# uc-vision/smart-tree

Measured on AMD Instinct MI355X. Metric: points/sec end-to-end (voxelize->sparse-UNet->skeleton), 1M-pt tree, higher is better.
Workload: dtype f32

## Files before the change

include/smarttree_hip.h:

```cpp
#ifndef SMARTTREE_HIP_H
#define SMARTTREE_HIP_H

#include <stdint.h>

#ifdef __cplusplus
extern "C" {
#endif

int st_version(void);
#define ST_SKELETON_STATS_ENTRIES 16
#define ST_SKELETON_TUNING_ENTRIES 24
int st_abi_entries(int what);
const char* st_last_error(void);
int64_t st_query_workspace(int op, int64_t a, int64_t b, int64_t c);

int64_t st_scan_workspace_bytes(int64_t n);
int st_scan_u32(const uint32_t* in, uint32_t* out, int64_t n, uint32_t* total, void* ws, int64_t ws_bytes, void* stream);
int64_t st_sort_workspace_bytes(int64_t n);
int st_sort_pairs_u32(uint32_t* keys, uint32_t* vals, int64_t n, int key_bits, void* ws, int64_t ws_bytes, void* stream);

int64_t st_voxelize_workspace_bytes(int64_t n_points, int max_blocks, int64_t max_voxels);
int st_voxelize_blocks(const float* xyz, const float* rgb, int64_t n, double voxel_size, double block_size,
                       double buffer_size, int min_points, int max_blocks, int64_t max_voxels, float* feats,
                       int32_t* coords, uint8_t* mask, int64_t* point_index, float* block_centres,
// ... 17 lines not shown
                              int32_t* up_order ,
                              void* stream);

int st_sparse_conv_fwd(const float* x0, int c0, const float* x1, int cin, const int32_t* nbr, int K, int64_t n_out,
                       const float* w, int cout, const float* scale, const float* shift, const float* residual,
                       int relu, float* y, const int32_t* row_order ,
                       void* stream, int64_t nbr_stride );
int st_sparse_conv_mfma_fwd(const float* x0, int c0, const float* x1, int cin, const int32_t* nbr, int K, int64_t n_out,
                            const float* wp, int cout, const float* scale, const float* shift, const float* residual,
                            int relu, float* y, const int32_t* row_order ,
                            void* stream, int64_t nbr_stride ,
                            int variant );
int st_sparse_conv_b3_fwd(const float* x0, int c0, const float* x1, int cin, const int32_t* nbr, int K, int64_t n_out, const void* wq,
                          int cout, const float* scale, const float* shift, const float* residual, int relu, float* y,
                          const int32_t* row_order, void* stream, int64_t nbr_stride, int variant);
int st_sparse_conv_f16_fwd(const void* x0, int c0, const void* x1, int cin, const int32_t* nbr, int K, int64_t n_out,
                           const void* w, int cout, const float* scale, const float* shift, const void* residual, int relu,
                           void* y, int in_half, int out_half, const int32_t* row_order, void* stream, int64_t nbr_stride );

int64_t st_brick_pyramid_workspace_bytes(int64_t n0, int n_blocks, int coord_bound, int depth, const int64_t* caps);
int st_brick_pyramid(const int32_t* coords0 , int64_t n0, int n_blocks ,
                     int coord_bound , int depth, const int32_t* blk_seg ,
                     int nseg, const int64_t* caps ,
                     int32_t* order0 , int32_t* const* coords_out ,
                     int32_t* const* subm , int32_t* const* down ,
                     int32_t* const* up , int32_t* const* up_order ,
                     int64_t* counts_host , void* ws, int64_t ws_bytes, void* stream);
int st_head_param_floats(void);
int st_pointwise_mlp_heads(const float* x, int64_t n, const float* params, float* radius, float* direction,
                           float* class_l, float* medial_vector , int64_t* class_idx , void* stream);
// ... 157 lines not shown
```

smart_tree_amd/_lib.py:

```python
from __future__ import annotations

import ctypes
from ctypes import c_double, c_float, c_int, c_int64, c_void_p
from pathlib import Path

import torch

_PKG = Path(__file__).resolve().parent
LIB_PATH = _PKG / "libsmarttree_hip.so"

_LIB = None
_ALLOW_HOST_POINTERS = False

P = c_void_p
I64 = c_int64

SIGNATURES = {
    "st_version": (c_int, []),
    "st_abi_entries": (c_int, [c_int]),
    "st_last_error": (ctypes.c_char_p, []),
    "st_scan_workspace_bytes": (I64, [I64]),
    "st_scan_u32": (c_int, [P, P, I64, P, P, I64, P]),
    "st_sort_workspace_bytes": (I64, [I64]),
    "st_sort_pairs_u32": (c_int, [P, P, I64, c_int, P, I64, P]),
# ... 1 lines not shown
    "st_voxelize_blocks": (c_int, [P, P, I64, c_double, c_double, c_double, c_int, c_int, I64, P, P, P, P, P,
                                   ctypes.POINTER(I64), ctypes.POINTER(I64), P, I64, P]),
    "st_hash_capacity": (I64, [I64]),
    "st_build_coord_hash": (c_int, [P, I64, P, P, I64, P]),
    "st_build_subm_rulebook": (c_int, [P, I64, P, P, I64, P, P]),
    "st_strided_workspace_bytes": (I64, [I64]),
    "st_spatial_order_workspace_bytes": (I64, [I64]),
    "st_spatial_order": (c_int, [P, I64, P, P, I64, P]),
    "st_move_rows": (c_int, [P, c_int, P, I64, P, c_int, P]),
    "st_build_strided_outputs": (c_int, [P, I64, I64, P, P, P, I64, ctypes.POINTER(I64), ctypes.POINTER(ctypes.c_int32),
                                         P, I64, P]),
    "st_build_strided_rulebook": (c_int, [P, I64, P, P, I64, P, I64, P, P, I64, ctypes.POINTER(ctypes.c_int32), P, P, P, P]),
    "st_sparse_conv_fwd": (c_int, [P, c_int, P, c_int, P, c_int, I64, P, c_int, P, P, P, c_int, P, P, P, I64]),
    "st_sparse_conv_mfma_fwd": (c_int, [P, c_int, P, c_int, P, c_int, I64, P, c_int, P, P, P, c_int, P, P, P, I64, c_int]),
    "st_sparse_conv_b3_fwd": (c_int, [P, c_int, P, c_int, P, c_int, I64, P, c_int, P, P, P, c_int, P, P, P, I64, c_int]),
    "st_sparse_conv_f16_fwd": (c_int, [P, c_int, P, c_int, P, c_int, I64, P, c_int, P, P, P, c_int, P, c_int, c_int, P, P, I64]),
    "st_brick_pyramid_workspace_bytes": (I64, [I64, c_int, c_int, c_int, ctypes.POINTER(I64)]),
    "st_brick_pyramid": (c_int, [P, I64, c_int, c_int, c_int, P, c_int, ctypes.POINTER(I64), P, ctypes.POINTER(P), ctypes.POINTER(P),
                                 ctypes.POINTER(P), ctypes.POINTER(P), ctypes.POINTER(P), ctypes.POINTER(I64), P, I64, P]),
    "st_head_param_floats": (c_int, []),
    "st_pointwise_mlp_heads": (c_int, [P, I64, P, P, P, P, P, P, P]),
    "st_knn_workspace_bytes": (I64, [I64]),
    "st_knn_radius": (c_int, [P, I64, P, I64, c_int, c_float, P, c_int, c_float, P, P, P, I64, P]),
    "st_medial_points": (c_int, [P, P, I64, P, P, P]),
    "st_centre_cloud": (c_int, [P, I64, P, P, I64, P]),
    "st_make_edges_workspace_bytes": (I64, [I64]),
    "st_make_edges": (c_int, [P, P, I64, c_int, P, P, ctypes.POINTER(I64), P, I64, P]),
    "st_connected_components_workspace_bytes": (c_int64, [c_int64]),
    "st_connected_components": (c_int, [P, I64, I64, P, P, I64, P]),
    "st_component_layout_workspace_bytes": (I64, [I64]),
# ... 48 lines not shown
    "st_bn_stats": (c_int, [P, c_int, I64, c_int, P, P, I64, P]),
    "st_bn_apply": (c_int, [P, c_int, I64, c_int, P, P, P, P, P, P]),
    "st_bn_backward_stats": (c_int, [P, P, c_int, I64, c_int, P, P, P, P, I64, P]),
    "st_bn_backward_apply": (c_int, [P, P, c_int, I64, c_int, P, P, P, P, P, P, P]),
    "st_skeleton_components": (c_int, [c_int, P, P, I64, P, P, P, P, P, P, c_float, c_int, c_int, P, P, P, P, P, P, P, P,
                                       P, P, ctypes.POINTER(I64), P, I64, P]),
}


ENQUEUE_ONLY = frozenset({
    "st_version", "st_abi_entries", "st_last_error", "st_scan_workspace_bytes", "st_sort_workspace_bytes", "st_voxelize_workspace_bytes",
    "st_hash_capacity", "st_strided_workspace_bytes", "st_head_param_floats", "st_knn_workspace_bytes",
    "st_make_edges_workspace_bytes", "st_connected_components_workspace_bytes", "st_component_layout_workspace_bytes",
    "st_component_csr_workspace_bytes", "st_assemble_workspace_bytes", "st_skeleton_workspace_bytes",
    "st_build_coord_hash", "st_build_subm_rulebook", "st_build_strided_rulebook", "st_sparse_conv_fwd",
    "st_sparse_conv_mfma_fwd", "st_sparse_conv_b3_fwd", "st_sparse_conv_f16_fwd", "st_pointwise_mlp_heads", "st_medial_points", "st_centre_cloud",
    "st_connected_components", "st_component_csr", "st_post_process", "st_knn_radius", "st_brick_pyramid_workspace_bytes",
    "st_centre_cloud_seg", "st_centre_cloud_box_seg", "st_voxelize_workspace_bytes_seg", "st_build_strided_rulebook_seg", "st_knn_workspace_bytes_seg",
    "st_knn_radius_seg", "st_skeleton_workspace_bytes_seg", "st_post_process_seg", "st_radius_count_seg",
    "st_voxelize_cloud_workspace_bytes", "st_loss_workspace_bytes", "st_spatial_order_workspace_bytes", "st_spatial_order", "st_connected_components_knn", "st_component_csr_knn", "st_component_csr_knn_workspace_bytes", "st_move_rows",
    "st_loss_backward", "st_sparse_conv_wgrad_workspace_bytes", "st_sparse_conv_wgrad",
    "st_sparse_conv_h_fwd", "st_sparse_conv_wgrad_h_workspace_bytes", "st_sparse_conv_wgrad_h", "st_move_rows_h",
    "st_bn_workspace_bytes", "st_bn_stats", "st_bn_apply", "st_bn_backward_stats", "st_bn_backward_apply",
    "st_sample_tubes_workspace_bytes", "st_sample_tubes_fill", "st_skeleton_match_workspace_bytes", "st_skeleton_match",
})


NOWAIT_VARIANTS = ("st_make_edges", "st_assemble_branches", "st_make_edges_seg")


class _Bound:
# ... 79 lines not shown
```

smart_tree_amd/csrc/sparse_conv.hip:

```cpp
#include "st_common.h"

#define CONV_BLOCK 256

typedef _Float16 st_h;
typedef _Float16 st_v4h __attribute__((ext_vector_type(4)));
__device__ __forceinline__ float4 conv_load4(const float* p) { return *reinterpret_cast<const float4*>(p); }
__device__ __forceinline__ float4 conv_load4(const st_h* p) {
    const st_v4h v = *reinterpret_cast<const st_v4h*>(p);
    return make_float4((float)v.x, (float)v.y, (float)v.z, (float)v.w);
}
__device__ __forceinline__ void conv_store4(float* p, float a, float b, float c, float d) { *reinterpret_cast<float4*>(p) = make_float4(a, b, c, d); }
__device__ __forceinline__ void conv_store4(st_h* p, float a, float b, float c, float d) {
    *reinterpret_cast<st_v4h*>(p) = st_v4h{(st_h)a, (st_h)b, (st_h)c, (st_h)d};
}

__device__ __forceinline__ uint32_t conv_live_offsets(int32_t entry, int K) {
    const uint32_t tag = (uint32_t)entry >> 28;
    if (!(tag & 8u) || K != 27) return 0xffffffffu;
    const uint32_t ax[3] = {(tag & 4u) ? 5u : 2u, (tag & 2u) ? 5u : 2u, (tag & 1u) ? 5u : 2u};
    uint32_t live = 0;
#pragma unroll
    for (int k = 0; k < 27; k++)
        if (((ax[0] >> (k / 9)) & (ax[1] >> ((k / 3) % 3)) & (ax[2] >> (k % 3))) & 1u) live |= 1u << k;
    return live;
}
#define CONV_ROW_MASK 0x0fffffff

template <int CIN, int COT, class TIN = float, class TOUT = float>
__global__ void __launch_bounds__(CONV_BLOCK) k_sparse_conv(const TIN* __restrict__ x0, int c0,
                                                            const TIN* __restrict__ x1, const int32_t* __restrict__ nbr,
                                                            int K, int64_t n_out, int64_t nstride, const float* __restrict__ w, int cout,
                                                            const float* __restrict__ scale, const float* __restrict__ shift,
                                                            const float* __restrict__ residual, int relu,
                                                            TOUT* __restrict__ y, const int32_t* __restrict__ row_order) {
    const int co_tiles = cout / COT;
    const int co0 = (int)(blockIdx.x % co_tiles) * COT;
    const int64_t pos = (int64_t)(blockIdx.x / co_tiles) * CONV_BLOCK + threadIdx.x;
    const bool active = pos < n_out;
    const int32_t entry = active && row_order ? row_order[pos] : 0;
    const int64_t o = active && row_order ? (int64_t)(entry & CONV_ROW_MASK) : pos;
    const uint32_t live = conv_live_offsets(entry, K);
    const int c1 = CIN - c0;
    float acc[COT];
#pragma unroll
    for (int c = 0; c < COT; c++) acc[c] = 0.0f;

    if (CIN % 4 == 0 && CIN <= 16) {
        constexpr int G = CIN <= 8 ? 9 : 3, Q = CIN / 4;
        for (int k0 = 0; k0 < K; k0 += G) {
            int idx[G];
            float4 v[G][Q];
#pragma unroll
            for (int j = 0; j < G; j++) {
                const int k = k0 + j;
                idx[j] = -1;
                if (k < K && active && ((live >> k) & 1u)) idx[j] = nbr ? nbr[(int64_t)k * nstride + o] : (int)o;
            }
#pragma unroll
            for (int j = 0; j < G; j++)
                if (idx[j] >= 0) {
#pragma unroll
                    for (int q = 0; q < Q; q++) {
                        const int ci = 4 * q;
                        const TIN* row = ci < c0 ? x0 + (int64_t)idx[j] * c0 + ci : x1 + (int64_t)idx[j] * c1 + (ci - c0);
                        v[j][q] = conv_load4(row);
                    }
                }
#pragma unroll
            for (int j = 0; j < G; j++) {
                if (idx[j] < 0) continue;
                const float* __restrict__ wk = w + (int64_t)(k0 + j) * CIN * cout + co0;
#pragma unroll
                for (int q = 0; q < Q; q++) {
                    const float xs[4] = {v[j][q].x, v[j][q].y, v[j][q].z, v[j][q].w};
#pragma unroll
                    for (int jj = 0; jj < 4; jj++)
#pragma unroll
                        for (int c = 0; c < COT; c++) acc[c] = fmaf(xs[jj], wk[(4 * q + jj) * cout + c], acc[c]);
                }
            }
        }
    } else
    for (int k = 0; k < K; k++) {
        int idx = -1;
        if (active && ((live >> k) & 1u)) idx = nbr ? nbr[(int64_t)k * nstride + o] : (int)o;
        if (idx < 0) continue;
        const float* __restrict__ wk = w + (int64_t)k * CIN * cout + co0;
        if (CIN % 4 == 0) {
#pragma unroll 2
            for (int ci = 0; ci < CIN; ci += 4) {
                const TIN* row = ci < c0 ? x0 + (int64_t)idx * c0 + ci : x1 + (int64_t)idx * c1 + (ci - c0);
                const float4 v = conv_load4(row);
                const float xs[4] = {v.x, v.y, v.z, v.w};
#pragma unroll
                for (int j = 0; j < 4; j++)
#pragma unroll
                    for (int c = 0; c < COT; c++) acc[c] = fmaf(xs[j], wk[(ci + j) * cout + c], acc[c]);
            }
        } else {
            for (int ci = 0; ci < CIN; ci++) {
// ... 8 lines not shown
    for (int c = 0; c < COT; c++) {
        float v = acc[c];
        if (scale) v = fmaf(v, scale[co0 + c], shift[co0 + c]);
        if (residual) v += residual[o * cout + co0 + c];
        if (relu) v = v > 0.0f ? v : 0.0f;
        acc[c] = v;
    }
    TOUT* out = y + o * cout + co0;
    if (COT % 4 == 0) {
#pragma unroll
        for (int c = 0; c < COT; c += 4) conv_store4(out + c, acc[c], acc[c + 1], acc[c + 2], acc[c + 3]);
    } else {
#pragma unroll
        for (int c = 0; c < COT; c++) out[c] = (TOUT)acc[c];
    }
}

__global__ void __launch_bounds__(CONV_BLOCK) k_sparse_conv_any(const float* __restrict__ x0, int c0, const float* __restrict__ x1, int cin,
                                                                const int32_t* __restrict__ nbr, int K, int64_t n_out, int64_t nstride,
                                                                const float* __restrict__ w, int cout, const float* __restrict__ scale,
                                                                const float* __restrict__ shift, const float* __restrict__ residual, int relu,
                                                                float* __restrict__ y, const int32_t* __restrict__ row_order) {
    const int64_t pos = (int64_t)blockIdx.x * CONV_BLOCK + threadIdx.x;
    if (pos >= n_out) return;
    const int co0 = (int)blockIdx.y * 4, nco = cout - co0 < 4 ? cout - co0 : 4;
    const int32_t entry = row_order ? row_order[pos] : 0;
    const int64_t o = row_order ? (int64_t)(entry & CONV_ROW_MASK) : pos;
    const uint32_t live = conv_live_offsets(entry, K);
    const int c1 = cin - c0;
    float acc[4] = {0.0f, 0.0f, 0.0f, 0.0f};
// ... 18 lines not shown

struct ConvArgs {
    const void* x0;
    int c0;
    const void* x1;
    const int32_t* nbr;
    int K;
    int64_t n_out, nstride;
    const void* w;
    const float *scale, *shift;
    const void* residual;
    int relu;
    void* y;
    const int32_t* row_order;
    hipStream_t stream;
};

static int conv_check_args(ConvArgs* a, int cin) {
    if (a->nstride <= 0) a->nstride = a->n_out;
    ST_REQUIRE(a->K >= 1 && (a->nbr != nullptr || a->K == 1), "conv: a NULL neighbour table means pointwise (K = 1)");
    ST_REQUIRE(a->c0 > 0 && a->c0 <= cin && (a->c0 == cin || a->x1 != nullptr), "conv: bad concat split");
    ST_REQUIRE((a->scale == nullptr) == (a->shift == nullptr), "conv: scale and shift go together");
    return ST_OK;
}

template <int CIN, int COT, class TIN = float, class TOUT = float>
static int conv_launch(const ConvArgs& a, int cout) {
    int64_t blocks = st_div_up(a.n_out, CONV_BLOCK) * (cout / COT);
    hipLaunchKernelGGL((k_sparse_conv<CIN, COT, TIN, TOUT>), dim3((unsigned)blocks), dim3(CONV_BLOCK), 0, a.stream, (const TIN*)a.x0, a.c0,
                       (const TIN*)a.x1, a.nbr, a.K, a.n_out, a.nstride, (const float*)a.w, cout, a.scale, a.shift, (const float*)a.residual,
// ... 73 lines not shown
    static constexpr int CHUNK = 32, PLANES = 1;
    typedef st_v8h Row;
    static __device__ __forceinline__ Row no_row() { return Row{}; }
    static __device__ __forceinline__ Row load_row(const T* row) { return *reinterpret_cast<const st_v8h*>(row); }
    static __device__ __forceinline__ A fragment(const Row& r) { return r; }
    static __device__ __forceinline__ B load_b(const W* wc, int) { return *wc; }
    static __device__ __forceinline__ void mma(const A& a, const B& b, st_v4f& d) { d = __builtin_amdgcn_mfma_f32_16x16x32_f16(a, b, d, 0, 0, 0); }
};

#define MF_PARAMS(T, W)                                                                                                               \
    const T *__restrict__ x0, int c0, const T *__restrict__ x1, const int32_t *__restrict__ nbr, int K, int64_t n_out, int64_t nstride, \
        const W *__restrict__ w, const float *__restrict__ scale, const float *__restrict__ shift, const T *__restrict__ residual,     \
        int relu, T *__restrict__ y, const int32_t *__restrict__ row_order
#define MF_ARGS x0, c0, x1, nbr, K, n_out, nstride, w, scale, shift, residual, relu, y, row_order

template <class OP, int CIN, int COUT, int RT, bool LDSW>
__device__ __forceinline__ void conv_rule_gemm(MF_PARAMS(typename OP::T, typename OP::W)) {
    typedef typename OP::T T;
    typedef typename OP::W W;
    constexpr bool PAIR = CIN == 16 && OP::CHUNK == 32;
    constexpr int CT = COUT / 16, NC = PAIR ? 1 : CIN / OP::CHUNK, LCH = OP::CHUNK / 4;
    constexpr int PLANE = 4 * COUT, WSTEP = NC * OP::PLANES * PLANE;
    __shared__ W wl[LDSW ? WSTEP : 1];
    const int tid = threadIdx.x, lane = tid & 63, wave = tid >> 6;
    const int i16 = lane & 15, g = lane >> 4;
    const int64_t obase = ((int64_t)blockIdx.x * (MF_BLOCK / 64) + wave) * (16 * RT);
    const int c1 = CIN - c0;
    st_v4f acc[RT][CT];
#pragma unroll
    for (int t = 0; t < RT; t++)
#pragma unroll
        for (int ct = 0; ct < CT; ct++) acc[t][ct] = st_v4f{0.0f, 0.0f, 0.0f, 0.0f};
// ... 50 lines not shown
        const float sc = scale ? scale[ch] : 1.0f, sh = scale ? shift[ch] : 0.0f;
#pragma unroll
        for (int t = 0; t < RT; t++)
#pragma unroll
            for (int r = 0; r < 4; r++) {
                const int64_t pos = obase + t * 16 + g * 4 + r;
                if (pos >= n_out) continue;
                const int64_t o = row_order ? (int64_t)(row_order[pos] & CONV_ROW_MASK) : pos;
                float v = acc[t][ct][r];
                if (scale) v = fmaf(v, sc, sh);
                if (residual) v += (float)residual[o * COUT + ch];
                if (relu) v = v > 0.0f ? v : 0.0f;
                y[o * COUT + ch] = (T)v;
            }
    }
}

template <int CIN, int COUT, int RT, bool LDSW>
__global__ void __launch_bounds__(MF_BLOCK) k_sparse_conv_mfma(MF_PARAMS(float, float4)) { conv_rule_gemm<MfF32, CIN, COUT, RT, LDSW>(MF_ARGS); }
template <int CIN, int COUT, int RT>
__global__ void __launch_bounds__(MF_BLOCK) k_sparse_conv_mfma_b3(MF_PARAMS(float, uint4)) { conv_rule_gemm<MfB3, CIN, COUT, RT, false>(MF_ARGS); }
template <int COUT, int RT>
__global__ void __launch_bounds__(MF_BLOCK) k_sparse_conv_mfma_b3_c16(MF_PARAMS(float, uint4)) { conv_rule_gemm<MfB3, 16, COUT, RT, false>(MF_ARGS); }
template <int CIN, int COUT, int RT>
__global__ void __launch_bounds__(MF_BLOCK) k_sparse_conv_mfma_f16x(MF_PARAMS(st_h, st_v8h)) { conv_rule_gemm<MfF16, CIN, COUT, RT, false>(MF_ARGS); }
template <int COUT, int RT>
__global__ void __launch_bounds__(MF_BLOCK) k_sparse_conv_mfma_f16x_c16(MF_PARAMS(st_h, st_v8h)) { conv_rule_gemm<MfF16, 16, COUT, RT, false>(MF_ARGS); }

template <class T, class W>
using mf_kernel_t = void (*)(MF_PARAMS(T, W));
template <int CIN, int COUT, int RT>
static mf_kernel_t<float, uint4> b3_kernel() {
    if constexpr (CIN == 16) return k_sparse_conv_mfma_b3_c16<COUT, RT>;
    else return k_sparse_conv_mfma_b3<CIN, COUT, RT>;
}
template <int CIN, int COUT, int RT>
static mf_kernel_t<st_h, st_v8h> f16x_kernel() {
    if constexpr (CIN == 16) return k_sparse_conv_mfma_f16x_c16<COUT, RT>;
    else return k_sparse_conv_mfma_f16x<CIN, COUT, RT>;
}

template <class T, class W>
static int mf_launch(mf_kernel_t<T, W> kernel, int rt, const ConvArgs& a) {
    hipLaunchKernelGGL(kernel, dim3((unsigned)st_div_up(a.n_out, (MF_BLOCK / 64) * 16 * rt)), dim3(MF_BLOCK), 0, a.stream, (const T*)a.x0, a.c0,
                       (const T*)a.x1, a.nbr, a.K, a.n_out, a.nstride, (const W*)a.w, a.scale, a.shift, (const T*)a.residual, a.relu, (T*)a.y,
                       a.row_order);
    ST_CHECK_LAUNCH();
    return ST_OK;
}

static int conv_row_tiles(const ConvArgs& a) { return a.n_out >= (a.row_order == nullptr ? 56000 : 300000) ? 2 : 1; }

template <int CIN, int COUT>
static int conv_launch_mfma(const ConvArgs& a, int v) {
    if (v == 0) v = (a.row_order == nullptr && a.n_out >= 150000) ? 18 : 1;
    switch (v) {
        case 1: return mf_launch(k_sparse_conv_mfma<CIN, COUT, 1, false>, 1, a);
        case 2: return mf_launch(k_sparse_conv_mfma<CIN, COUT, 2, false>, 2, a);
        case 4: return mf_launch(k_sparse_conv_mfma<CIN, COUT, 4, false>, 4, a);
        case 17: return mf_launch(k_sparse_conv_mfma<CIN, COUT, 1, true>, 1, a);
        default: return mf_launch(k_sparse_conv_mfma<CIN, COUT, 2, true>, 2, a);
// ... 8 lines not shown
    ST_REQUIRE((cin % 32 == 0 || (cin == 16 && c0 == cin)) && cout % 16 == 0 && c0 % 8 == 0,
               "conv(b3): Cin % 32 (or Cin = 16 without concat), Cout % 16 and a concat split % 8 are required");
    if (n_out <= 0) return ST_OK;
    const int rt = variant == 1 || variant == 2 ? variant : conv_row_tiles(a);
#define B3_CASE(CI, CO) \
    if (cin == CI && cout == CO) return rt == 2 ? mf_launch(b3_kernel<CI, CO, 2>(), 2, a) : mf_launch(b3_kernel<CI, CO, 1>(), 1, a);
    B3_CASE(16, 16)
    B3_CASE(16, 32)
    B3_CASE(32, 16)
    B3_CASE(32, 32)
    B3_CASE(32, 64)
    B3_CASE(64, 32)
    B3_CASE(64, 64)
#undef B3_CASE
    st_set_error("conv(b3): no kernel instance for cin=%d cout=%d", cin, cout);
    return ST_ERR_INVALID;
}

extern "C" int st_sparse_conv_f16_fwd(const void* x0, int c0, const void* x1, int cin, const int32_t* nbr, int K, int64_t n_out,
                                      const void* w, int cout, const float* scale, const float* shift, const void* residual,
                                      int relu, void* y, int in_half, int out_half, const int32_t* row_order, void* stream_,
                                      int64_t nbr_stride) {
    ConvArgs a = {x0, c0, x1, nbr, K, n_out, nbr_stride, w, scale, shift, residual, relu, y, row_order, (hipStream_t)stream_};
    ST_TRY(conv_check_args(&a, cin));
    ST_REQUIRE(in_half || out_half, "conv(f16): neither side is half precision -- use st_sparse_conv_fwd");
    if (n_out <= 0) return ST_OK;
    if (in_half && out_half) {
        ST_REQUIRE(cin % 16 == 0 && cout % 16 == 0 && c0 % 16 == 0, "conv(f16): channels and concat split must be multiples of 16");
        const int rt = conv_row_tiles(a);
#define F16X_CASE(CI, CO) \
// ... 60 lines not shown
    CONV_CASE(16, 8, 8)
    CONV_CASE(16, 16, 16)
    CONV_CASE(16, 32, 16)
    CONV_CASE(32, 16, 16)
    CONV_CASE(32, 32, 16)
    CONV_CASE(32, 64, 16)
    CONV_CASE(64, 32, 16)
    CONV_CASE(64, 64, 16)
#undef CONV_CASE
    hipLaunchKernelGGL(k_sparse_conv_any, dim3((unsigned)st_div_up(n_out, CONV_BLOCK), (unsigned)st_div_up(cout, 4)), dim3(CONV_BLOCK), 0, a.stream, x0, c0,
                       x1, cin, nbr, K, n_out, a.nstride, w, cout, scale, shift, residual, relu, y, row_order);
    ST_CHECK_LAUNCH();
    return ST_OK;
}

#define HEAD_W1 0
#define HEAD_S1 64
#define HEAD_T1 72
#define HEAD_W2 80
#define HEAD_S2 112
#define HEAD_T2 116
#define HEAD_W3 120
#define HEAD_STRIDE 132

template <int NOUT>
__device__ __forceinline__ void head_eval(const float* __restrict__ p, const float* x, float* out) {
    float h1[8], h2[4];
#pragma unroll
    for (int co = 0; co < 8; co++) {
        float a = 0.0f;
// ... 60 lines not shown
```

smart_tree_amd/model/model.py:

```python
from __future__ import annotations

import contextlib

from typing import Dict, Mapping

import numpy as np
import torch

from . import sparse_ops as ops
from .. import profiling

BN_EPS = 1e-4


def _conv_weight(t: torch.Tensor) -> torch.Tensor:
    cout, cin = t.shape[0], t.shape[-1]
    return t.reshape(cout, -1, cin).permute(1, 2, 0).contiguous().float()


class _Affine:

    def __init__(self, sd: Mapping[str, torch.Tensor], prefix: str, device):
        g = sd[prefix + ".weight"].double()
        b = sd[prefix + ".bias"].double()
# ... 37 lines not shown
                        self.wp16[name] = ops.mfma_weight16_half(self.w[name])
            elif key.endswith(".running_mean") and "_head." not in key:
                p = key[: -len(".running_mean")]
                self.bn[p] = _Affine(sd, p, self.device)
        self.generic_heads = not self._heads_are_standard(sd)
        self.head_params = None if self.generic_heads else self._pack_heads(sd).to(self.device)
        if self.generic_heads:
            self.head_layers = {}
            for name in ("radius_head", "direction_head", "class_head"):
                mat = lambda i: sd[f"{name}.sequence.{i}.weight"].reshape(sd[f"{name}.sequence.{i}.weight"].shape[0], -1).T.contiguous().float()
                self.head_layers[name] = [(mat(0).unsqueeze(0).to(self.device), _Affine(sd, f"{name}.sequence.1", self.device)),
                                          (mat(3).unsqueeze(0).to(self.device), _Affine(sd, f"{name}.sequence.4", self.device)),
                                          (mat(6).unsqueeze(0).to(self.device), None)]
        self.use_bricks = True
        self.spatial_order = True
        self.trace = None

    def eval(self):
        return self

    def to(self, device):
        return self if torch.device(device) == self.device else Smart_Tree(self._state, device, self.fp16)

    @staticmethod
    def _heads_are_standard(sd) -> bool:
        for name, nout in (("radius_head", 1), ("direction_head", 3), ("class_head", 2)):
            shapes = [tuple(sd[f"{name}.sequence.{i}.weight"].reshape(sd[f"{name}.sequence.{i}.weight"].shape[0], -1).shape) for i in (0, 3, 6)]
            if shapes != [(8, 8), (4, 8), (nout, 4)]:
                return False
        return True
# ... 29 lines not shown
            s2, t2 = affine(4)
            w3 = torch.zeros(12, dtype=torch.float64)
            w3[: 4 * nout] = mat(6).reshape(-1)
            blocks.append(torch.cat([mat(0).reshape(-1), s1, t1, mat(3).reshape(-1), s2, t2, w3]))
        return torch.cat(blocks).float().contiguous()

    def _conv(self, name, x, nbr, n_out, x1=None, bn=None, residual=None, relu=False, row_order=None):
        a = self.bn[bn] if bn else None
        out_half = self.fp16 and self.w[name].shape[2] % 16 == 0
        return ops.sparse_conv(x, self.w[name], nbr, n_out, x1=x1, scale=a.scale if a else None,
                               shift=a.shift if a else None, residual=residual, relu=relu,
                               wp=self.wp.get(name) if self.use_mfma else None, out_half=out_half,
                               wp16=self.wp16.get(name), row_order=row_order,
                               wq=self.wq.get(name) if self.use_mfma and self.use_b3 and not self.fp16 else None)

    def _res_block(self, prefix, x, nbr, x1=None):
        n = x.shape[0]
        h = self._conv(prefix + ".sequence.0", x, nbr, n, x1=x1, bn=prefix + ".sequence.1", relu=True)
        ident = self._conv(prefix + ".identity.0", x, None, n, x1=x1) if x1 is not None else x
        return self._conv(prefix + ".sequence.3", h, nbr, n, bn=prefix + ".sequence.4", residual=ident, relu=True)

    def _ublock(self, prefix, x, pyr, level):
        x = self._res_block(prefix + ".Head", x, pyr.subm[level])
        self._record(f"head{level}", x)
        if level == self.depth:
            return x
        n_fine, n_coarse = x.shape[0], pyr.coords[level + 1].shape[0]
        z = self._conv(prefix + ".Encode.sequence.0", x, pyr.down[level], n_coarse, bn=prefix + ".Encode.sequence.1",
                       relu=True)
        self._record(f"enc{level}", z)
        z = self._ublock(prefix + ".U", z, pyr, level + 1)
        d = self._conv(prefix + ".Decode.sequence.0", z, pyr.up[level], n_fine, bn=prefix + ".Decode.sequence.1",
                       relu=True, row_order=pyr.up_order[level] if pyr.up_order else None)
        self._record(f"dec{level}", d)
        x = self._res_block(prefix + ".Tail", x, pyr.subm[level], x1=d)
        self._record(f"tail{level}", x)
        return x

    def _record(self, name, x):
        if self.trace is not None:
            self.trace[name] = x

    def features(self, sparse_input):
        coords = sparse_input.indices.contiguous()
        feats = sparse_input.features.contiguous().float()
        blk_seg, n_seg = getattr(sparse_input, "blk_seg", None), getattr(sparse_input, "n_seg", 1)
        reorder = self.spatial_order and self.trace is None and coords.shape[0] > 1
        hint = getattr(sparse_input, "brick_hint", None)
        bricks = ops.brick_pyramid(coords, self.depth, hint[0], hint[1], blk_seg, n_seg) if reorder and hint and self.use_bricks else None
        if bricks is not None:
            pyr, order = bricks
            feats = ops.move_rows(feats, order)
        else:
            order = ops.spatial_order(coords) if reorder else None
            if order is not None:
                coords, feats = ops.move_rows(coords, order), ops.move_rows(feats, order)
            pyr = ops.build_pyramid(coords, self.depth, blk_seg, n_seg)
        gate = getattr(self, "conv_gate", None)
        with (gate() if gate is not None else contextlib.nullcontext()), profiling.kernel_family("k_sparse_conv* (one forward pass)"):
            x = self._conv("input_conv.sequence.0", feats, None, feats.shape[0], bn="input_conv.sequence.1", relu=True)
            self._record("input", x)
            x = self._ublock("UNet", x, pyr, 0)
        if order is not None:
            x = ops.move_rows(x, order, scatter=True)
        return x

    def forward(self, sparse_input) -> Dict[str, torch.Tensor]:
        x = self.features(sparse_input)
        radius, direction, class_l, _, _ = self._generic_heads(x, False) if self.generic_heads else ops.mlp_heads(x, self.head_params)
        return {"radius": radius, "direction": direction, "class_l": class_l}

    __call__ = forward

    def forward_fused_tail(self, sparse_input):
        x = self.features(sparse_input)
        return self._generic_heads(x, True) if self.generic_heads else ops.mlp_heads(x, self.head_params, with_tail=True)
```

smart_tree_amd/model/sparse_ops.py:

```python
from __future__ import annotations

import ctypes
from dataclasses import dataclass, field
from typing import List, Optional

import torch

from .. import _lib, profiling


@dataclass
class CoordHash:
    keys: torch.Tensor
    vals: torch.Tensor
    cap: int


def build_coord_hash(coords: torch.Tensor) -> CoordHash:
    L = _lib.lib()
    n = coords.shape[0]
    cap = L.st_hash_capacity(n)
    keys = torch.empty(cap, dtype=torch.int64, device=coords.device)
    vals = torch.empty(cap, dtype=torch.int32, device=coords.device)
    _lib.check(L.st_build_coord_hash(_lib.ptr(coords), n, _lib.ptr(keys), _lib.ptr(vals), cap, _lib.stream(coords.device)))
# ... 282 lines not shown
    elif wp is not None and mfma_eligible(cin, cout, c0) and not big_16:
        entry, wt, name, tail = L.st_sparse_conv_mfma_fwd, wp, f"k_sparse_conv_mfma<{cin},{cout}>", (int(MFMA_VARIANT),)
    else:
        entry, wt, name = L.st_sparse_conv_fwd, w, f"k_sparse_conv<{cin},{cout}>"
    esz_in, esz_out = (2 if in_half else 4), (2 if out_half else 4)
    y = torch.empty((n_out, cout), dtype=torch.float16 if out_half else torch.float32, device=x0.device)
    nbytes = (lambda: (_pair_count(nbr) if nbr is not None else n_out) * (cin * esz_in + (4 if nbr is not None else 0))
              + n_out * cout * esz_out) if profiling.enabled() else 0
    nflops = (lambda: 2.0 * (_pair_count(nbr) if nbr is not None else n_out) * cin * cout) if profiling.enabled() else 0
    with profiling.kernel(name + ("" if nbr is not None else " k1"), nbytes, nflops):
        _lib.check(entry(_lib.ptr(x0), c0, _lib.ptr(x1), cin, nbr_ptr, K, n_out, _lib.ptr(wt), cout, _lib.ptr(scale), _lib.ptr(shift),
                         _lib.ptr(residual), int(relu), _lib.ptr(y), *mid, _lib.ptr(row_order), _lib.stream(x0.device), nbr_stride, *tail))
    return y


_pairs_cache = {}


def _pair_count(nbr: torch.Tensor) -> int:
    key = (id(nbr), profiling.generation())
    if key not in _pairs_cache:
        if len(_pairs_cache) > 4096:
            _pairs_cache.clear()
        _pairs_cache[key] = int((nbr >= 0).sum().item())
    return _pairs_cache[key]


def mlp_heads(x: torch.Tensor, params: torch.Tensor, with_tail: bool = False):
    L = _lib.lib()
    n, dev = x.shape[0], x.device
# ... 11 lines not shown
```

Measured before the change: 937.4 million.

## Fuse Tail identity projection into first conv and fold input gather into input conv

Adds fused kernels in which the Tail residual block's 1x1 identity projection of the concatenated (skip, decoded) features is computed inside the first submanifold conv kernel, for both the vector and b3 MFMA paths. It also adds an input-conv kernel that reads the unpermuted features through the spatial order instead of running a separate move_rows. Together these remove extra launches and re-reads of the concatenated rows. The cost is more register pressure and longer kernels, and the fused path is only taken on the b3/MFMA fp32 path when no trace is recorded.

Result: no change. 938.9 million, median of 4 (+0.2%).

```diff
diff --git a/include/smarttree_hip.h b/include/smarttree_hip.h
--- a/include/smarttree_hip.h
+++ b/include/smarttree_hip.h
@@ -55,6 +55,15 @@
 int st_sparse_conv_b3_fwd(const float* x0, int c0, const float* x1, int cin, const int32_t* nbr, int K, int64_t n_out, const void* wq,
                           int cout, const float* scale, const float* shift, const float* residual, int relu, float* y,
                           const int32_t* row_order, void* stream, int64_t nbr_stride, int variant);
+int st_sparse_conv_tail_fwd(const float* x0, int c0, const float* x1, int cin, const int32_t* nbr, int K, int64_t n_out,
+                            const float* w, int cout, const float* scale, const float* shift, const float* residual, int relu,
+                            float* y, const int32_t* row_order, void* stream, int64_t nbr_stride, const float* w_ident, float* y_ident);
+int st_sparse_conv_tail_b3_fwd(const float* x0, int c0, const float* x1, int cin, const int32_t* nbr, int K, int64_t n_out,
+                               const void* wq, int cout, const float* scale, const float* shift, const float* residual, int relu,
+                               float* y, const int32_t* row_order, void* stream, int64_t nbr_stride, int variant,
+                               const void* wq_ident, float* y_ident);
+int st_sparse_conv_input_fwd(const float* x0, int cin, int64_t n_out, const float* w, int cout, const float* scale,
+                             const float* shift, int relu, float* y, const int32_t* in_order, void* stream);
 int st_sparse_conv_f16_fwd(const void* x0, int c0, const void* x1, int cin, const int32_t* nbr, int K, int64_t n_out,
                            const void* w, int cout, const float* scale, const float* shift, const void* residual, int relu,
                            void* y, int in_half, int out_half, const int32_t* row_order, void* stream, int64_t nbr_stride );
diff --git a/smart_tree_amd/_lib.py b/smart_tree_amd/_lib.py
--- a/smart_tree_amd/_lib.py
+++ b/smart_tree_amd/_lib.py
@@ -39,6 +39,9 @@
     "st_sparse_conv_fwd": (c_int, [P, c_int, P, c_int, P, c_int, I64, P, c_int, P, P, P, c_int, P, P, P, I64]),
     "st_sparse_conv_mfma_fwd": (c_int, [P, c_int, P, c_int, P, c_int, I64, P, c_int, P, P, P, c_int, P, P, P, I64, c_int]),
     "st_sparse_conv_b3_fwd": (c_int, [P, c_int, P, c_int, P, c_int, I64, P, c_int, P, P, P, c_int, P, P, P, I64, c_int]),
+    "st_sparse_conv_tail_fwd": (c_int, [P, c_int, P, c_int, P, c_int, I64, P, c_int, P, P, P, c_int, P, P, P, I64, P, P]),
+    "st_sparse_conv_tail_b3_fwd": (c_int, [P, c_int, P, c_int, P, c_int, I64, P, c_int, P, P, P, c_int, P, P, P, I64, c_int, P, P]),
+    "st_sparse_conv_input_fwd": (c_int, [P, c_int, I64, P, c_int, P, P, c_int, P, P, P]),
     "st_sparse_conv_f16_fwd": (c_int, [P, c_int, P, c_int, P, c_int, I64, P, c_int, P, P, P, c_int, P, c_int, c_int, P, P, I64]),
     "st_brick_pyramid_workspace_bytes": (I64, [I64, c_int, c_int, c_int, ctypes.POINTER(I64)]),
     "st_brick_pyramid": (c_int, [P, I64, c_int, c_int, c_int, P, c_int, ctypes.POINTER(I64), P, ctypes.POINTER(P), ctypes.POINTER(P),
@@ -117,7 +120,8 @@
     "st_make_edges_workspace_bytes", "st_connected_components_workspace_bytes", "st_component_layout_workspace_bytes",
     "st_component_csr_workspace_bytes", "st_assemble_workspace_bytes", "st_skeleton_workspace_bytes",
     "st_build_coord_hash", "st_build_subm_rulebook", "st_build_strided_rulebook", "st_sparse_conv_fwd",
-    "st_sparse_conv_mfma_fwd", "st_sparse_conv_b3_fwd", "st_sparse_conv_f16_fwd", "st_pointwise_mlp_heads", "st_medial_points", "st_centre_cloud",
+    "st_sparse_conv_mfma_fwd", "st_sparse_conv_b3_fwd", "st_sparse_conv_f16_fwd", "st_pointwise_mlp_heads", "st_medial_points",
+    "st_sparse_conv_tail_fwd", "st_sparse_conv_tail_b3_fwd", "st_sparse_conv_input_fwd", "st_centre_cloud",
     "st_connected_components", "st_component_csr", "st_post_process", "st_knn_radius", "st_brick_pyramid_workspace_bytes",
     "st_centre_cloud_seg", "st_centre_cloud_box_seg", "st_voxelize_workspace_bytes_seg", "st_build_strided_rulebook_seg", "st_knn_workspace_bytes_seg",
     "st_knn_radius_seg", "st_skeleton_workspace_bytes_seg", "st_post_process_seg", "st_radius_count_seg",
diff --git a/smart_tree_amd/csrc/sparse_conv.hip b/smart_tree_amd/csrc/sparse_conv.hip
--- a/smart_tree_amd/csrc/sparse_conv.hip
+++ b/smart_tree_amd/csrc/sparse_conv.hip
@@ -26,13 +26,17 @@
 }
 #define CONV_ROW_MASK 0x0fffffff
 
-template <int CIN, int COT, class TIN = float, class TOUT = float>
-__global__ void __launch_bounds__(CONV_BLOCK) k_sparse_conv(const TIN* __restrict__ x0, int c0,
-                                                            const TIN* __restrict__ x1, const int32_t* __restrict__ nbr,
-                                                            int K, int64_t n_out, int64_t nstride, const float* __restrict__ w, int cout,
-                                                            const float* __restrict__ scale, const float* __restrict__ shift,
-                                                            const float* __restrict__ residual, int relu,
-                                                            TOUT* __restrict__ y, const int32_t* __restrict__ row_order) {
+#define CONV_PARAMS(TIN, TOUT)                                                                                                    \
+    const TIN *__restrict__ x0, int c0, const TIN *__restrict__ x1, const int32_t *__restrict__ nbr, int K, int64_t n_out,        \
+        int64_t nstride, const float *__restrict__ w, int cout, const float *__restrict__ scale, const float *__restrict__ shift, \
+        const float *__restrict__ residual, int relu, TOUT *__restrict__ y, const int32_t *__restrict__ row_order
+#define CONV_ARGS x0, c0, x1, nbr, K, n_out, nstride, w, cout, scale, shift, residual, relu, y, row_order
+
+enum { CONV_PLAIN = 0, CONV_TAIL = 1, CONV_INPUT = 2 };
+
+template <int CIN, int COT, class TIN, class TOUT, int MODE>
+__device__ __forceinline__ void conv_vector(CONV_PARAMS(TIN, TOUT), const float* __restrict__ w_id, TOUT* __restrict__ y_id,
+                                            const int32_t* __restrict__ in_order) {
     const int co_tiles = cout / COT;
     const int co0 = (int)(blockIdx.x % co_tiles) * COT;
     const int64_t pos = (int64_t)(blockIdx.x / co_tiles) * CONV_BLOCK + threadIdx.x;
@@ -41,7 +45,30 @@
     const int64_t o = active && row_order ? (int64_t)(entry & CONV_ROW_MASK) : pos;
     const uint32_t live = conv_live_offsets(entry, K);
     const int c1 = CIN - c0;
+    const int self = MODE == CONV_INPUT ? (active ? in_order[o] : 0) : (int)o;
     float acc[COT];
+    if (MODE == CONV_TAIL && active) {
+        static_assert(MODE != CONV_TAIL || CIN % 4 == 0, "the fused identity reads the concatenated row in float4 pieces");
+#pragma unroll
+        for (int c = 0; c < COT; c++) acc[c] = 0.0f;
+#pragma unroll
+        for (int ci = 0; ci < CIN; ci += 4) {
+            const float4 v = conv_load4(ci < c0 ? x0 + o * c0 + ci : x1 + o * c1 + (ci - c0));
+            const float xs[4] = {v.x, v.y, v.z, v.w};
+#pragma unroll
+            for (int j = 0; j < 4; j++)
+#pragma unroll
+                for (int c = 0; c < COT; c++) acc[c] = fmaf(xs[j], w_id[(ci + j) * cout + co0 + c], acc[c]);
+        }
+        TOUT* out = y_id + o * cout + co0;
+        if (COT % 4 == 0) {
+#pragma unroll
+            for (int c = 0; c < COT; c += 4) conv_store4(out + c, acc[c], acc[c + 1], acc[c + 2], acc[c + 3]);
+        } else {
+#pragma unroll
+            for (int c = 0; c < COT; c++) out[c] = (TOUT)acc[c];
+        }
+    }
 #pragma unroll
     for (int c = 0; c < COT; c++) acc[c] = 0.0f;
 
@@ -54,7 +81,7 @@
             for (int j = 0; j < G; j++) {
                 const int k = k0 + j;
                 idx[j] = -1;
-                if (k < K && active && ((live >> k) & 1u)) idx[j] = nbr ? nbr[(int64_t)k * nstride + o] : (int)o;
+                if (k < K && active && ((live >> k) & 1u)) idx[j] = nbr ? nbr[(int64_t)k * nstride + o] : self;
             }
 #pragma unroll
             for (int j = 0; j < G; j++)
@@ -83,7 +110,7 @@
     } else
     for (int k = 0; k < K; k++) {
         int idx = -1;
-        if (active && ((live >> k) & 1u)) idx = nbr ? nbr[(int64_t)k * nstride + o] : (int)o;
+        if (active && ((live >> k) & 1u)) idx = nbr ? nbr[(int64_t)k * nstride + o] : self;
         if (idx < 0) continue;
         const float* __restrict__ wk = w + (int64_t)k * CIN * cout + co0;
         if (CIN % 4 == 0) {
@@ -122,6 +149,19 @@
 #pragma unroll
         for (int c = 0; c < COT; c++) out[c] = (TOUT)acc[c];
     }
+}
+
+template <int CIN, int COT, class TIN = float, class TOUT = float>
+__global__ void __launch_bounds__(CONV_BLOCK) k_sparse_conv(CONV_PARAMS(TIN, TOUT)) {
+    conv_vector<CIN, COT, TIN, TOUT, CONV_PLAIN>(CONV_ARGS, nullptr, nullptr, nullptr);
+}
+template <int CIN, int COT>
+__global__ void __launch_bounds__(CONV_BLOCK) k_sparse_conv_tail(CONV_PARAMS(float, float), const float* __restrict__ w_id, float* __restrict__ y_id) {
+    conv_vector<CIN, COT, float, float, CONV_TAIL>(CONV_ARGS, w_id, y_id, nullptr);
+}
+template <int CIN, int COT>
+__global__ void __launch_bounds__(CONV_BLOCK) k_sparse_conv_input(CONV_PARAMS(float, float), const int32_t* __restrict__ in_order) {
+    conv_vector<CIN, COT, float, float, CONV_INPUT>(CONV_ARGS, nullptr, nullptr, in_order);
 }
 
 __global__ void __launch_bounds__(CONV_BLOCK) k_sparse_conv_any(const float* __restrict__ x0, int c0, const float* __restrict__ x1, int cin,
@@ -170,6 +210,9 @@
     void* y;
     const int32_t* row_order;
     hipStream_t stream;
+    const void* w_id = nullptr;
+    void* y_id = nullptr;
+    const int32_t* in_order = nullptr;
 };
 
 static int conv_check_args(ConvArgs* a, int cin) {
@@ -273,8 +316,9 @@
         int relu, T *__restrict__ y, const int32_t *__restrict__ row_order
 #define MF_ARGS x0, c0, x1, nbr, K, n_out, nstride, w, scale, shift, residual, relu, y, row_order
 
-template <class OP, int CIN, int COUT, int RT, bool LDSW>
-__device__ __forceinline__ void conv_rule_gemm(MF_PARAMS(typename OP::T, typename OP::W)) {
+template <class OP, int CIN, int COUT, int RT, bool LDSW, bool TAIL = false>
+__device__ __forceinline__ void conv_rule_gemm(MF_PARAMS(typename OP::T, typename OP::W), const typename OP::W* __restrict__ w_id = nullptr,
+                                               typename OP::T* __restrict__ y_id = nullptr) {
     typedef typename OP::T T;
     typedef typename OP::W W;
     constexpr bool PAIR = CIN == 16 && OP::CHUNK == 32;
@@ -355,6 +399,42 @@
                 y[o * COUT + ch] = (T)v;
             }
     }
+    if constexpr (TAIL) {
+        static_assert(!PAIR && !LDSW, "the fused identity exists for the 32-channel-chunk instances without LDS staging");
+#pragma unroll
+        for (int t = 0; t < RT; t++)
+#pragma unroll
+            for (int ct = 0; ct < CT; ct++) acc[t][ct] = st_v4f{0.0f, 0.0f, 0.0f, 0.0f};
+#pragma unroll
+        for (int c = 0; c < NC; c++) {
+            const int ci = OP::CHUNK * c + LCH * g;
+            typename OP::A a[RT];
+#pragma unroll
+            for (int t = 0; t < RT; t++) {
+                typename OP::Row r = OP::no_row();
+                if (orow[t] >= 0) r = OP::load_row(ci < c0 ? x0 + orow[t] * c0 + ci : x1 + orow[t] * c1 + (ci - c0));
+                a[t] = OP::fragment(r);
+            }
+#pragma unroll
+            for (int ct = 0; ct < CT; ct++) {
+                const typename OP::B b = OP::load_b(w_id + (c * OP::PLANES * 4 + g) * COUT + ct * 16 + i16, PLANE);
+#pragma unroll
+                for (int t = 0; t < RT; t++) OP::mma(a[t], b, acc[t][ct]);
+            }
+        }
+#pragma unroll
+        for (int ct = 0; ct < CT; ct++)
+#pragma unroll
+            for (int t = 0; t < RT; t++) {
+#pragma unroll
+                for (int r = 0; r < 4; r++) {
+                    const int64_t pos = obase + t * 16 + g * 4 + r;
+                    if (pos >= n_out) continue;
+                    const int64_t o = row_order ? (int64_t)(row_order[pos] & CONV_ROW_MASK) : pos;
+                    y_id[o * COUT + ct * 16 + i16] = (T)acc[t][ct][r];
+                }
+            }
+    }
 }
 
 template <int CIN, int COUT, int RT, bool LDSW>
@@ -368,6 +448,11 @@
 template <int COUT, int RT>
 __global__ void __launch_bounds__(MF_BLOCK) k_sparse_conv_mfma_f16x_c16(MF_PARAMS(st_h, st_v8h)) { conv_rule_gemm<MfF16, 16, COUT, RT, false>(MF_ARGS); }
 
+template <int CIN, int COUT, int RT>
+__global__ void __launch_bounds__(MF_BLOCK) k_sparse_conv_tail_b3(MF_PARAMS(float, uint4), const uint4* __restrict__ w_id, float* __restrict__ y_id) {
+    conv_rule_gemm<MfB3, CIN, COUT, RT, false, true>(MF_ARGS, w_id, y_id);
+}
+
 template <class T, class W>
 using mf_kernel_t = void (*)(MF_PARAMS(T, W));
 template <int CIN, int COUT, int RT>
@@ -386,6 +471,14 @@
     hipLaunchKernelGGL(kernel, dim3((unsigned)st_div_up(a.n_out, (MF_BLOCK / 64) * 16 * rt)), dim3(MF_BLOCK), 0, a.stream, (const T*)a.x0, a.c0,
                        (const T*)a.x1, a.nbr, a.K, a.n_out, a.nstride, (const W*)a.w, a.scale, a.shift, (const T*)a.residual, a.relu, (T*)a.y,
                        a.row_order);
+    ST_CHECK_LAUNCH();
+    return ST_OK;
+}
+
+static int mf_launch_tail(void (*kernel)(MF_PARAMS(float, uint4), const uint4*, float*), int rt, const ConvArgs& a) {
+    hipLaunchKernelGGL(kernel, dim3((unsigned)st_div_up(a.n_out, (MF_BLOCK / 64) * 16 * rt)), dim3(MF_BLOCK), 0, a.stream, (const float*)a.x0, a.c0,
+                       (const float*)a.x1, a.nbr, a.K, a.n_out, a.nstride, (const uint4*)a.w, a.scale, a.shift, (const float*)a.residual, a.relu,
+                       (float*)a.y, a.row_order, (const uint4*)a.w_id, (float*)a.y_id);
     ST_CHECK_LAUNCH();
     return ST_OK;
 }
@@ -424,6 +517,22 @@
     B3_CASE(64, 64)
 #undef B3_CASE
     st_set_error("conv(b3): no kernel instance for cin=%d cout=%d", cin, cout);
+    return ST_ERR_INVALID;
+}
+
+extern "C" int st_sparse_conv_tail_b3_fwd(const float* x0, int c0, const float* x1, int cin, const int32_t* nbr, int K, int64_t n_out,
+                                          const void* wq, int cout, const float* scale, const float* shift, const float* residual,
+                                          int relu, float* y, const int32_t* row_order, void* stream_, int64_t nbr_stride, int variant,
+                                          const void* wq_ident, float* y_ident) {
+    ConvArgs a = {x0, c0, x1, nbr, K, n_out, nbr_stride, wq, scale, shift, residual, relu, y, row_order, (hipStream_t)stream_, wq_ident, y_ident};
+    ST_TRY(conv_check_args(&a, cin));
+    ST_REQUIRE(cin % 32 == 0 && cout % 16 == 0 && c0 % 8 == 0, "conv(tail b3): Cin % 32, Cout % 16 and a concat split % 8 are required");
+    ST_REQUIRE(wq_ident != nullptr && y_ident != nullptr && y_ident != y, "conv(tail b3): identity weights and an output of its own are required");
+    if (n_out <= 0) return ST_OK;
+    const int rt = variant == 1 || variant == 2 ? variant : conv_row_tiles(a);
+    if (cin == 32 && cout == 16) return rt == 2 ? mf_launch_tail(k_sparse_conv_tail_b3<32, 16, 2>, 2, a) : mf_launch_tail(k_sparse_conv_tail_b3<32, 16, 1>, 1, a);
+    if (cin == 64 && cout == 32) return rt == 2 ? mf_launch_tail(k_sparse_conv_tail_b3<64, 32, 2>, 2, a) : mf_launch_tail(k_sparse_conv_tail_b3<64, 32, 1>, 1, a);
+    st_set_error("conv(tail b3): no kernel instance for cin=%d cout=%d", cin, cout);
     return ST_ERR_INVALID;
 }
 
@@ -514,6 +623,35 @@
     return ST_OK;
 }
 
+extern "C" int st_sparse_conv_tail_fwd(const float* x0, int c0, const float* x1, int cin, const int32_t* nbr, int K, int64_t n_out,
+                                       const float* w, int cout, const float* scale, const float* shift, const float* residual, int relu,
+                                       float* y, const int32_t* row_order, void* stream_, int64_t nbr_stride, const float* w_ident,
+                                       float* y_ident) {
+    ConvArgs a = {x0, c0, x1, nbr, K, n_out, nbr_stride, w, scale, shift, residual, relu, y, row_order, (hipStream_t)stream_, w_ident, y_ident};
+    ST_TRY(conv_check_args(&a, cin));
+    ST_REQUIRE(w_ident != nullptr && y_ident != nullptr && y_ident != y, "conv(tail): identity weights and an output of its own are required");
+    ST_REQUIRE(cin == 16 && cout == 8 && c0 % 4 == 0, "conv(tail): the instance is cin = 16, cout = 8 with a concat split % 4");
+    if (n_out <= 0) return ST_OK;
+    hipLaunchKernelGGL((k_sparse_conv_tail<16, 8>), dim3((unsigned)st_div_up(n_out, CONV_BLOCK)), dim3(CONV_BLOCK), 0, a.stream, x0, c0, x1, nbr, K,
+                       n_out, a.nstride, w, cout, scale, shift, residual, relu, y, row_order, w_ident, y_ident);
+    ST_CHECK_LAUNCH();
+    return ST_OK;
+}
+
+extern "C" int st_sparse_conv_input_fwd(const float* x0, int cin, int64_t n_out, const float* w, int cout, const float* scale,
+                                        const float* shift, int relu, float* y, const int32_t* in_order, void* stream_) {
+    if (in_order == nullptr) return st_sparse_conv_fwd(x0, cin, nullptr, cin, nullptr, 1, n_out, w, cout, scale, shift, nullptr, relu, y, nullptr, stream_, 0);
+    ConvArgs a = {x0, cin, nullptr, nullptr, 1, n_out, 0, w, scale, shift, nullptr, relu, y, nullptr, (hipStream_t)stream_};
+    ST_TRY(conv_check_args(&a, cin));
+    ST_REQUIRE(cin == 3 && cout == 8, "conv(input): the instance is cin = 3, cout = 8");
+    if (n_out <= 0) return ST_OK;
+    hipLaunchKernelGGL((k_sparse_conv_input<3, 8>), dim3((unsigned)st_div_up(n_out, CONV_BLOCK)), dim3(CONV_BLOCK), 0, a.stream, x0, cin,
+                       (const float*)nullptr, (const int32_t*)nullptr, 1, n_out, a.nstride, w, cout, scale, shift, (const float*)nullptr, relu, y,
+                       (const int32_t*)nullptr, in_order);
+    ST_CHECK_LAUNCH();
+    return ST_OK;
+}
+
 #define HEAD_W1 0
 #define HEAD_S1 64
 #define HEAD_T1 72
diff --git a/smart_tree_amd/model/model.py b/smart_tree_amd/model/model.py
--- a/smart_tree_amd/model/model.py
+++ b/smart_tree_amd/model/model.py
@@ -75,6 +75,7 @@
                                           (mat(6).unsqueeze(0).to(self.device), None)]
         self.use_bricks = True
         self.spatial_order = True
+        self.fuse_pointwise = True
         self.trace = None
 
     def eval(self):
@@ -134,13 +135,21 @@
                                wp16=self.wp16.get(name), row_order=row_order,
                                wq=self.wq.get(name) if self.use_mfma and self.use_b3 and not self.fp16 else None)
 
-    def _res_block(self, prefix, x, nbr, x1=None):
+    def _fusing(self) -> bool:
+        return self.fuse_pointwise and self.use_mfma and self.use_b3 and not self.fp16 and self.trace is None
+
+    def _res_block(self, prefix, x, nbr, x1=None, fuse=False):
         n = x.shape[0]
-        h = self._conv(prefix + ".sequence.0", x, nbr, n, x1=x1, bn=prefix + ".sequence.1", relu=True)
-        ident = self._conv(prefix + ".identity.0", x, None, n, x1=x1) if x1 is not None else x
+        s0, idn = prefix + ".sequence.0", prefix + ".identity.0"
+        if x1 is not None and fuse and ops.tail_fusable(*self.w[s0].shape[1:], x.shape[1], self.wq.get(s0)):
+            a = self.bn[prefix + ".sequence.1"]
+            h, ident = ops.sparse_conv_tail(x, x1, self.w[s0], self.w[idn], nbr, n, a.scale, a.shift, self.wq.get(s0), self.wq.get(idn))
+        else:
+            h = self._conv(s0, x, nbr, n, x1=x1, bn=prefix + ".sequence.1", relu=True)
+            ident = self._conv(idn, x, None, n, x1=x1) if x1 is not None else x
         return self._conv(prefix + ".sequence.3", h, nbr, n, bn=prefix + ".sequence.4", residual=ident, relu=True)
 
-    def _ublock(self, prefix, x, pyr, level):
+    def _ublock(self, prefix, x, pyr, level, fuse=False):
         x = self._res_block(prefix + ".Head", x, pyr.subm[level])
         self._record(f"head{level}", x)
         if level == self.depth:
@@ -149,11 +158,11 @@
         z = self._conv(prefix + ".Encode.sequence.0", x, pyr.down[level], n_coarse, bn=prefix + ".Encode.sequence.1",
                        relu=True)
         self._record(f"enc{level}", z)
-        z = self._ublock(prefix + ".U", z, pyr, level + 1)
+        z = self._ublock(prefix + ".U", z, pyr, level + 1, fuse)
         d = self._conv(prefix + ".Decode.sequence.0", z, pyr.up[level], n_fine, bn=prefix + ".Decode.sequence.1",
                        relu=True, row_order=pyr.up_order[level] if pyr.up_order else None)
         self._record(f"dec{level}", d)
-        x = self._res_block(prefix + ".Tail", x, pyr.subm[level], x1=d)
+        x = self._res_block(prefix + ".Tail", x, pyr.subm[level], x1=d, fuse=fuse)
         self._record(f"tail{level}", x)
         return x
 
@@ -162,6 +171,9 @@
             self.trace[name] = x
 
     def features(self, sparse_input):
+        return self._features(sparse_input, False)
+
+    def _features(self, sparse_input, fuse):
         coords = sparse_input.indices.contiguous()
         feats = sparse_input.features.contiguous().float()
         blk_seg, n_seg = getattr(sparse_input, "blk_seg", None), getattr(sparse_input, "n_seg", 1)
@@ -170,28 +182,35 @@
         bricks = ops.brick_pyramid(coords, self.depth, hint[0], hint[1], blk_seg, n_seg) if reorder and hint and self.use_bricks else None
         if bricks is not None:
             pyr, order = bricks
-            feats = ops.move_rows(feats, order)
         else:
             order = ops.spatial_order(coords) if reorder else None
             if order is not None:
-                coords, feats = ops.move_rows(coords, order), ops.move_rows(feats, order)
+                coords = ops.move_rows(coords, order)
             pyr = ops.build_pyramid(coords, self.depth, blk_seg, n_seg)
+        w_in = self.w["input_conv.sequence.0"]
+        fold_in = order is not None and fuse and tuple(w_in.shape) == (1, 3, 8) and feats.shape[1] == 3
+        if order is not None and not fold_in:
+            feats = ops.move_rows(feats, order)
         gate = getattr(self, "conv_gate", None)
         with (gate() if gate is not None else contextlib.nullcontext()), profiling.kernel_family("k_sparse_conv* (one forward pass)"):
-            x = self._conv("input_conv.sequence.0", feats, None, feats.shape[0], bn="input_conv.sequence.1", relu=True)
+            if fold_in:
+                a = self.bn["input_conv.sequence.1"]
+                x = ops.input_conv(feats, w_in, a.scale, a.shift, order)
+            else:
+                x = self._conv("input_conv.sequence.0", feats, None, feats.shape[0], bn="input_conv.sequence.1", relu=True)
             self._record("input", x)
-            x = self._ublock("UNet", x, pyr, 0)
-        if order is not None:
-            x = ops.move_rows(x, order, scatter=True)
-        return x
+            x = self._ublock("UNet", x, pyr, 0, fuse)
+        return x if order is None else ops.move_rows(x, order, scatter=True)
+
+    def _heads(self, sparse_input, with_tail: bool):
+        x = self._features(sparse_input, self._fusing())
+        return self._generic_heads(x, with_tail) if self.generic_heads else ops.mlp_heads(x, self.head_params, with_tail=with_tail)
 
     def forward(self, sparse_input) -> Dict[str, torch.Tensor]:
-        x = self.features(sparse_input)
-        radius, direction, class_l, _, _ = self._generic_heads(x, False) if self.generic_heads else ops.mlp_heads(x, self.head_params)
+        radius, direction, class_l, _, _ = self._heads(sparse_input, False)
         return {"radius": radius, "direction": direction, "class_l": class_l}
 
     __call__ = forward
 
     def forward_fused_tail(self, sparse_input):
-        x = self.features(sparse_input)
-        return self._generic_heads(x, True) if self.generic_heads else ops.mlp_heads(x, self.head_params, with_tail=True)
+        return self._heads(sparse_input, True)
diff --git a/smart_tree_amd/model/sparse_ops.py b/smart_tree_amd/model/sparse_ops.py
--- a/smart_tree_amd/model/sparse_ops.py
+++ b/smart_tree_amd/model/sparse_ops.py
@@ -320,6 +320,52 @@
     return y
 
 
+def tail_fusable(cin: int, cout: int, c0: int, wq: Optional[torch.Tensor]) -> bool:
+    if (cin, cout) == (16, 8):
+        return c0 % 4 == 0
+    return wq is not None and (cin, cout) in ((32, 16), (64, 32)) and c0 % 8 == 0
+
+
+def sparse_conv_tail(x0: torch.Tensor, x1: torch.Tensor, w: torch.Tensor, w_ident: torch.Tensor, nbr: torch.Tensor, n_out: int,
+                     scale: torch.Tensor, shift: torch.Tensor, wq: Optional[torch.Tensor] = None,
+                     wq_ident: Optional[torch.Tensor] = None):
+    L = _lib.lib()
+    K, cin, cout = w.shape
+    c0 = x0.shape[1]
+    y = torch.empty((n_out, cout), dtype=torch.float32, device=x0.device)
+    y_ident = torch.empty((n_out, cout), dtype=torch.float32, device=x0.device)
+    if n_out == 0:
+        return y, y_ident
+    nbr_ptr, nbr_stride = _nbr_args(nbr)
+    b3 = (cin, cout) != (16, 8)
+    if not tail_fusable(cin, cout, c0, wq) or (b3 and wq_ident is None) or w_ident.shape != (1, cin, cout):
+        raise ValueError(f"no fused Tail kernel for cin={cin} cout={cout} c0={c0}")
+    nbytes = (lambda: _pair_count(nbr) * (cin * 4 + 4) + 2 * n_out * cout * 4) if profiling.enabled() else 0
+    nflops = (lambda: 2.0 * (_pair_count(nbr) + n_out) * cin * cout) if profiling.enabled() else 0
+    name = f"k_sparse_conv_tail_b3<{cin},{cout}>" if b3 else f"k_sparse_conv_tail<{cin},{cout}>"
+    with profiling.kernel(name, nbytes, nflops):
+        head = (_lib.ptr(x0), c0, _lib.ptr(x1), cin, nbr_ptr, K, n_out)
+        mid = (cout, _lib.ptr(scale), _lib.ptr(shift), None, 1, _lib.ptr(y), None, _lib.stream(x0.device), nbr_stride)
+        if b3:
+            _lib.check(L.st_sparse_conv_tail_b3_fwd(*head, _lib.ptr(wq), *mid, int(B3_VARIANT), _lib.ptr(wq_ident), _lib.ptr(y_ident)))
+        else:
+            _lib.check(L.st_sparse_conv_tail_fwd(*head, _lib.ptr(w), *mid, _lib.ptr(w_ident), _lib.ptr(y_ident)))
+    return y, y_ident
+
+
+def input_conv(x: torch.Tensor, w: torch.Tensor, scale: torch.Tensor, shift: torch.Tensor, in_order: torch.Tensor) -> torch.Tensor:
+    L = _lib.lib()
+    n, cin, cout = x.shape[0], w.shape[1], w.shape[2]
+    assert x.dtype == torch.float32 and in_order.dtype == torch.int32 and in_order.shape[0] == n
+    y = torch.empty((n, cout), dtype=torch.float32, device=x.device)
+    if n == 0:
+        return y
+    with profiling.kernel(f"k_sparse_conv_input<{cin},{cout}> k1", n * (cin + cout + 1) * 4, 2.0 * n * cin * cout):
+        _lib.check(L.st_sparse_conv_input_fwd(_lib.ptr(x), cin, n, _lib.ptr(w), cout, _lib.ptr(scale), _lib.ptr(shift), 1, _lib.ptr(y),
+                                              _lib.ptr(in_order), _lib.stream(x.device)))
+    return y
+
+
 _pairs_cache = {}
 
 
```
